# GMichailov/Flash-Attention-CUDA-C

Hardware: AMD Instinct MI355X
Metric: fwd attention TFLOP/s/GPU (bf16, seq=4096, d=128) + % MFMA peak (higher is better)
Workload: dtype bf16

## Files before the change

flash-attention-cuda-c_amd/csrc/computers.hip.h:

```cpp
#pragma once

#include "slot_engine.hip.h"

namespace fa {

template <int R>
struct Scores {
    f32x16 s[R][2];
};

template <class C>
struct WaveCompute : SlotEngine<WaveCompute<C>, C> {
    static constexpr int D = C::D, ESZ = C::ESZ, R = 1;
    static constexpr int KS = D / 16;
    static constexpr int DB = D / 32;
    static constexpr int NA = 2 * KS, NB = 4 * DB;
    static constexpr int SA = NA * R, SB = NB * R;
    static constexpr int MPF = ESZ == 1 ? 2 : 1;
    static constexpr int NF = NA / MPF;
    static constexpr int FPH = NF / 2;
    static constexpr int NPRE = C::NPRE < NF ? C::NPRE : NF;
    static constexpr int VPRE = C::VPRE;
    static constexpr int GROUPS = R, RG = 32, LOG_RG = 5, FPG = FPH;
    static constexpr int NE = 32 * R;
    static constexpr int SPAN = SA + (3 * SB) / 4;
    using G = TileGeom<D, ESZ>;
    using Stage = std::conditional_t<C::MIX, MixStage<D, C::NWAVES>,
                  std::conditional_t<C::DMA, DmaStage<D, C::NWAVES, false, true>,
                                     std::conditional_t<C::DMA_K8, HybridStageFp8<D, C::NWAVES>, BufStage<D, ESZ, C::NWAVES, C::PAD>>>>;
    using ScoresT = Scores<R>;
    static constexpr int NL = Stage::NL, NW = Stage::NW;

    u32x4 qf[R][FPH];
    f32x16 o[R][DB];
    float m[R];
    float l[R];
    u32x4 kf[NPRE];
    bf16x8 vf[VPRE + 1];
    uint32_t pw[R][16];
    float sum_a[R], sum_b[R], mx_a[R], mx_b[R], p_even, p_last;
    bool need;
    unsigned long long t_mid = 0, t_end = 0;

    __device__ __forceinline__ void init() {
#pragma unroll
        for (int r = 0; r < R; ++r) {
#pragma unroll
            for (int i = 0; i < DB; ++i)
#pragma unroll
                for (int k = 0; k < 16; ++k) o[r][i][k] = 0.f;
            m[r] = -INFINITY;
            l[r] = 0.f;
        }
// ... 14 lines not shown
            if constexpr ((F & 1) && SUB == MPF - 1) acc = mfma_32x32x64_fp8_unit_scale(kprev, kfrag, qf[RG][(F - 1) % FPH], q, acc);
        } else {
            static_assert(ESZ == 2, "the non-scaled form is for bf16 inputs");
            acc = mfma_32x32x16(__builtin_bit_cast(bf16x8, kfrag), __builtin_bit_cast(bf16x8, q), acc);
        }
    }
    __device__ __forceinline__ static void zero(Scores<R>& n) {
#pragma unroll
        for (int r = 0; r < R; ++r)
#pragma unroll
            for (int k = 0; k < 16; ++k) { n.s[r][0][k] = 0.f; n.s[r][1][k] = 0.f; }
    }

    template <int I = 0>
    __device__ __forceinline__ void qk_all(lds_ptr kimg, int kbase, Scores<R>& n) {
        if constexpr (I == 0) zero(n);
        if constexpr (I < SA) {
            constexpr int f = I / (MPF * R), sub = (I % (MPF * R)) / R, rg = I % R;
            if constexpr (I % (MPF * R) == 0) kf[f % 2] = k_read(kimg, kbase, f);
            qk_mfma<f, sub, rg>(kf[(f + 1) % 2], kf[f % 2], n);
            qk_all<I + 1>(kimg, kbase, n);
        }
    }

    __device__ __forceinline__ void mask(Scores<R>& n, int kv0, int q_row0, int S, int lane) const {
        const int k0 = kv0 + 4 * (lane >> 5);
#pragma unroll
        for (int r = 0; r < R; ++r) {
            const int qi = q_row0 + 32 * r + (lane & 31);
            const int lim = C::CAUSAL ? (qi < S - 1 ? qi : S - 1) : S - 1;
#pragma unroll
            for (int k = 0; k < 16; ++k) {
                n.s[r][0][k] = (k0 + acc_row(k, 0)) > lim ? -INFINITY : n.s[r][0][k];
                n.s[r][1][k] = (k0 + 32 + acc_row(k, 0)) > lim ? -INFINITY : n.s[r][1][k];
            }
        }
// ... 98 lines not shown
                constexpr int vn = v + VPRE;
                vf[vn % (VPRE + 1)] = v_frag(v_cur, vbase, vn / DB, vn % DB);
            }
            this->template exp_slot<SA + J, F16W>(cur, c);
            if constexpr (TRACK && J < SB / 2) max3_slot<J>(nxt);
            if constexpr (TRACK && J == SB / 2) this->decide(c);
            this->template write_in_slot<J, F16W>(st, wr_slot);
            __builtin_amdgcn_sched_barrier(0);
            slots_b<TRACK, J + 1, F16W>(st, wr_slot, v_cur, vbase, c, cur, nxt);
        }
    }

    __host__ __device__ static constexpr int tail_elem_slot(int E) { return (E / 8 - 1) * DB + (E % 8) * DB / 8; }
    template <int E, bool F16W = false>
    __device__ __forceinline__ void tail_pre(Stage& st, int t_load, lds_ptr v_cur, int vbase, float c, const Scores<R>& cur) {
        static_assert(R == 1 && NL <= 8 && VPRE <= DB, "tail step: one row group, the lead-in carries every piece");
        if constexpr (E < 8) {
            if constexpr (E < VPRE) vf[E % (VPRE + 1)] = v_frag(v_cur, vbase, E / DB, E % DB);
            if constexpr (E < NL) st.template load<E, F16W>(t_load);
            this->template exp_elem<E, F16W>(cur, c);
            tail_pre<E + 1, F16W>(st, t_load, v_cur, vbase, c, cur);
        }
    }
    template <int J, int ST, int E = 8, bool F16W = false>
    __device__ __forceinline__ void tail_exp(const Scores<R>& cur, float c) {
        if constexpr (E < 8 * (ST / DB)) {
            if constexpr (tail_elem_slot(E) == J) this->template exp_elem<E, F16W>(cur, c);
            tail_exp<J, ST, E + 1, F16W>(cur, c);
        }
    }
    template <int J, int J1, int ST, bool F16W = false>
    __device__ __forceinline__ void slots_t(lds_ptr v_cur, int vbase, float c, const Scores<R>& cur) {
        if constexpr (J < J1) {
            constexpr int s4 = J / DB, db = J % DB;
            if constexpr (F16W) o[0][db] = mfma_32x32x16(__builtin_bit_cast(f16x8, vf[J % (VPRE + 1)]), __builtin_bit_cast(f16x8, p_frag(0, s4)), o[0][db]);
            else o[0][db] = mfma_32x32x16(vf[J % (VPRE + 1)], p_frag(0, s4), o[0][db]);
            if constexpr (J + VPRE < ST) {
                constexpr int vn = J + VPRE;
                vf[vn % (VPRE + 1)] = v_frag(v_cur, vbase, vn / DB, vn % DB);
            }
            tail_exp<J, ST, 8, F16W>(cur, c);
            __builtin_amdgcn_sched_barrier(0);
            slots_t<J + 1, J1, ST, F16W>(v_cur, vbase, c, cur);
        }
    }
    __device__ __forceinline__ void begin_tail(Stage& st, lds_ptr wr_slot) {
        st.set_dst(wr_slot);
#pragma unroll
        for (int r = 0; r < R; ++r) sum_a[r] = sum_b[r] = 0.f;
    }

    __device__ __forceinline__ void begin_tile(Stage& st, lds_ptr wr_slot, Scores<R>& nxt) {
        st.set_dst(wr_slot);
#pragma unroll
        for (int r = 0; r < R; ++r) {
            sum_a[r] = sum_b[r] = 0.f;
            mx_a[r] = mx_b[r] = -INFINITY;
        }
// ... 17 lines not shown

    __device__ __forceinline__ bool not_finite() const {
        float acc[4] = {0.f, 0.f, 0.f, 0.f};
#pragma unroll
        for (int r = 0; r < R; ++r) {
            acc[0] = fmaf(l[r], 0.f, acc[0]);
#pragma unroll
            for (int i = 0; i < DB; ++i)
#pragma unroll
                for (int k = 0; k < 16; ++k) acc[k & 3] = fmaf(o[r][i][k], 0.f, acc[k & 3]);
        }
        const float a = (acc[0] + acc[1]) + (acc[2] + acc[3]);
        return a != a;
    }

    template <typename OutT>
    __device__ __forceinline__ void store_o_lds(lds_ptr region, char* Oh, float* lse_head, int64_t oS_bytes, int row0, int S,
                                                int lane, int orow_bytes = D * 2) {
        static_assert(sizeof(OutT) == 2, "LDS epilogue is for bf16 / f16 outputs");
        constexpr int ROWB = D * 2, CHUNKS = ROWB / 16;
        const int q = lane & 31, h = lane >> 5;
#pragma unroll
        for (int r = 0; r < R; ++r) {
            const float l_tot = sum_both_halves(l[r]);
            this->store_lse(lse_head, l_tot, r, row0, S, lane);
            const float inv = 1.0f / l_tot;
#pragma unroll
            for (int db = 0; db < DB; ++db)
#pragma unroll
                for (int g4 = 0; g4 < 4; ++g4) {
                    const int d0 = 32 * db + 8 * g4 + 4 * h;
                    const float a = o[r][db][4 * g4 + 0] * inv, b = o[r][db][4 * g4 + 1] * inv;
                    const float c2 = o[r][db][4 * g4 + 2] * inv, e = o[r][db][4 * g4 + 3] * inv;
                    u32x2 v;
                    if constexpr (__is_same(OutT, __bf16)) v = u32x2{pack_bf16(a, b), pack_bf16(c2, e)};
                    else v = u32x2{pack_f16(a, b), pack_f16(c2, e)};
                    const int chunk = (d0 * 2) >> 4, half8 = (d0 * 2) & 8;
                    *reinterpret_cast<FA_LDS u32x2*>(region + (32 * r + q) * ROWB + (((chunk ^ q) & (CHUNKS - 1)) << 4) + half8) = v;
                }
        }
        __builtin_amdgcn_s_waitcnt(0xc07f);
        constexpr int ROWS_PER_INST = 64 / CHUNKS;
        const int rr = lane / CHUNKS, cc = lane % CHUNKS;
        if (!C::PAD && row0 + 32 * R <= S) {
            u32x4 v[32 * R / ROWS_PER_INST];
#pragma unroll
            for (int i = 0; i < 32 * R / ROWS_PER_INST; ++i) {
                const int row = i * ROWS_PER_INST + rr;
                v[i] = *reinterpret_cast<FA_LDS const u32x4*>(region + row * ROWB + (((cc ^ row) & (CHUNKS - 1)) << 4));
            }
#pragma unroll
            for (int i = 0; i < 32 * R / ROWS_PER_INST; ++i)
                store_global_b128<C::O_CACHE>(Oh + (int64_t)(row0 + i * ROWS_PER_INST + rr) * oS_bytes + cc * 16, v[i]);
            return;
        }
#pragma unroll
        for (int i = 0; i < 32 * R / ROWS_PER_INST; ++i) {
            const int row = i * ROWS_PER_INST + rr;
            const u32x4 v = *reinterpret_cast<FA_LDS const u32x4*>(region + row * ROWB + (((cc ^ row) & (CHUNKS - 1)) << 4));
            if (row0 + row < S && (!C::PAD || cc * 16 < orow_bytes))
                *reinterpret_cast<u32x4*>(Oh + (int64_t)(row0 + row) * oS_bytes + cc * 16) = v;
        }
    }
    template <typename OutT>
    __device__ __forceinline__ void store_o_lds32(lds_ptr region, char* Oh, float* lse_head, int64_t oS_bytes, int row0, int S,
                                                  int lane, int orow_bytes = D * 4) {
        static_assert(sizeof(OutT) == 4, "for fp32 outputs");
        const int q = lane & 31, h = lane >> 5;
        float inv[R];
#pragma unroll
        for (int r = 0; r < R; ++r) {
            const float l_tot = sum_both_halves(l[r]);
            this->store_lse(lse_head, l_tot, r, row0, S, lane);
            inv[r] = 1.0f / l_tot;
        }
        const int rr = lane >> 4, cc = lane & 15;
#pragma unroll
        for (int hf = 0; hf < D / 64; ++hf) {
            if (hf > 0) __builtin_amdgcn_s_waitcnt(0xc07f);
#pragma unroll
            for (int r = 0; r < R; ++r)
#pragma unroll
                for (int dd = 0; dd < 2; ++dd)
#pragma unroll
                    for (int g4 = 0; g4 < 4; ++g4) {
                        const int db = 2 * hf + dd, cidx = 8 * dd + 2 * g4 + h;
                        const f32x4 v = {o[r][db][4 * g4 + 0] * inv[r], o[r][db][4 * g4 + 1] * inv[r],
                                         o[r][db][4 * g4 + 2] * inv[r], o[r][db][4 * g4 + 3] * inv[r]};
                        *reinterpret_cast<FA_LDS f32x4*>(region + (32 * r + q) * 256 + (((cidx ^ q) & 15) << 4)) = v;
                    }
            __builtin_amdgcn_s_waitcnt(0xc07f);
// ... 21 lines not shown
```

flash-attention-cuda-c_amd/csrc/kernel_bf16.hip.h:

```cpp
#pragma once

#include "computers.hip.h"
#include "computers16.hip.h"

#include <type_traits>

namespace fa {

struct Opt {
    bool stamp = false;
    bool pad = false;
    int m16 = -1;
    int sum_mfma = -1;
    int waves = 8;
    bool p_f16 = false;
    bool mix = false;
    int kv_clamp = -1;
    int q_nt = -1;
    int tail = -1;
    int tail_half = -1;
};

template <int D_, bool CAUSAL_, typename OutT_, int ESZ_ = 2, Opt O = Opt{}>
struct KernelCfg {
    static constexpr int D = D_;
    static constexpr bool CAUSAL = CAUSAL_;
    using OutT = OutT_;
    static constexpr int ESZ = ESZ_;
    static constexpr bool STAMP = O.stamp, PAD = O.pad;
    static constexpr bool PRIO_A = true;
    static constexpr int O_CACHE = CAUSAL_ ? 2 : 0;
    static constexpr int Q_CACHE = (O.q_nt < 0 ? CAUSAL_ : O.q_nt != 0) ? 2 : 0;
    static constexpr bool KV_CLAMP = CAUSAL_ && O.kv_clamp != 0;
    static constexpr bool TAIL = ESZ_ == 2 && O.m16 == 0 && (O.tail < 0 ? CAUSAL_ && O.mix : O.tail != 0);
    static constexpr bool TAIL_HALF = TAIL && CAUSAL_ && O.tail_half != 0;
    static constexpr bool COALESCED_Q = D_ == 128 && !O.pad;
    static constexpr bool MXQK = ESZ_ == 1;
    static constexpr bool M16 = (O.m16 < 0 ? true : O.m16 != 0) && ESZ_ == 2;
    static constexpr bool SUM_MFMA = M16 && (O.sum_mfma < 0 ? true : O.sum_mfma != 0);
    static constexpr bool VALU_FIRST = !M16;
    static constexpr bool P_F16 = M16 && O.p_f16;
    static constexpr bool LATE_ADD = !M16;
    static constexpr bool DMA = ESZ_ == 2 && !O.pad && !O.p_f16;
    static constexpr bool MIX = O.mix && DMA;
    static_assert(!O.mix || (ESZ_ == 2 && !O.pad && !O.p_f16 && (O.m16 == 0 || O.sum_mfma == 0)),
                  "the mixed-precision kernels are the LDS-DMA kernels (16x16x32 engine: with fp32 row sums)");
    static constexpr bool DMA_K8 = ESZ_ == 1 && D_ == 128 && !O.pad && O.waves == 8;
    static constexpr int NPRE = 4;
    static constexpr int VPRE = 2;
    static constexpr int THR = 8;
    static constexpr int NWAVES = O.waves;
    static_assert(NWAVES == 8 || NWAVES == 4, "8 or 4 waves");
    static constexpr int QBLK = 32 * NWAVES;
    static constexpr int RING = 3;
    static constexpr int RING_BYTES = RING * TileGeom<D_, ESZ_>::SLOT;
    static constexpr int EP_OFF = (DMA || DMA_K8) ? TileGeom<D_, ESZ_>::SLOT : 0;
    static constexpr int EP_NEED = EP_OFF + (sizeof(OutT_) == 2 ? QBLK * D_ * 2 : QBLK * 256);
    static constexpr int FLAG_OFF = EP_NEED > RING_BYTES ? EP_NEED : RING_BYTES;
    static constexpr int LDS_BYTES = FLAG_OFF + 64;
    static_assert(LDS_BYTES <= 163840, "160 KiB of LDS per CU");
};

template <int D, bool CAUSAL, typename OutT, int ESZ = 2, bool STAMP = false, bool PAD = false, bool LSE = false>
using ProdCfg = KernelCfg<D, CAUSAL, OutT, ESZ, Opt{.stamp = STAMP, .pad = PAD, .m16 = CAUSAL ? 0 : -1, .sum_mfma = LSE ? 0 : -1}>;
// ... 6 lines not shown
    u32x4 a = *reinterpret_cast<FA_LDS const u32x4*>(flags);
    uint32_t r = a[0] | a[1] | a[2] | a[3];
    if constexpr (NWAVES == 8) {
        const u32x4 b = *reinterpret_cast<FA_LDS const u32x4*>(flags + 16);
        r |= b[0] | b[1] | b[2] | b[3];
    }
    return __builtin_amdgcn_readfirstlane(r) != 0;
}

template <int D, typename OutT, bool STAMP = false>
using MixCfg = KernelCfg<D, true, OutT, 2, Opt{.stamp = STAMP, .m16 = 0, .mix = true}>;

template <class C>
using WaveComputeOf = std::conditional_t<C::M16, WaveCompute16<C>, WaveCompute<C>>;

template <class C, bool TRACK, bool F16W = C::P_F16>
__device__ __forceinline__ bool attention_pass(const Params& p, WaveComputeOf<C>& w, typename WaveComputeOf<C>::Stage& st, lds_ptr smem,
                                               int n_tiles, int my_tiles, int q_row0, int lane,
                                               unsigned long long (&acc)[24], bool tile0_in_flight) {
    using G = TileGeom<C::D, C::ESZ>;
    constexpr bool CAUSAL = C::CAUSAL;
    constexpr int KVBLK = 64, SLOT = G::SLOT, KT = G::K_TILE;
    const int S = p.Sk;
    unsigned long long tp0 = 0, tp1 = 0, tp2 = 0;
    if constexpr (C::STAMP) tp0 = cycle_stamp();
    w.init();
    using WC = WaveComputeOf<C>;
    constexpr int KBLK = (G::ROWB / 16) * 128;
    const int kbase = WC::Stage::K_DMA ? (C::M16 ? kd16_read_base(lane, KBLK) : kd_read_base(lane, KBLK)) : (C::M16 ? k16_read_base(lane) : k_read_base(lane));
    const int vbase = C::M16 ? v16_read_base<C::D>(lane) : v_read_base(lane);
    const float c = p.scale_log2;
    auto needs_mask = [&](int t) { return (CAUSAL && t * KVBLK + KVBLK - 1 > q_row0) || (t * KVBLK + KVBLK > S); };
    typename WC::ScoresT sA, sB;

    if (!tile0_in_flight) st.template load_all_into<F16W>(0, smem);
    st.template write_all<F16W>(smem);
    unsigned long long tw0 = 0;
    if constexpr (C::STAMP) tw0 = cycle_stamp();
    st.wait_all();
    if constexpr (C::STAMP) acc[16] += cycle_stamp() - tw0;
    __syncthreads();
    st.template load_all_into<F16W>(1, smem + SLOT);
    constexpr int AHEAD = C::RING - 1;
    if constexpr (C::STAMP) tp1 = cycle_stamp();
    if (my_tiles > 0) {
        w.qk_all(smem, kbase, sA);
        if (needs_mask(0)) w.mask(sA, 0, q_row0, S, lane);
        w.first_max(sA, c);
    }
    st.template write_all<F16W>(smem + SLOT);
    st.wait_all();
    __syncthreads();
    if constexpr (C::STAMP) { tp2 = cycle_stamp(); acc[8] += tp1 - tp0; acc[9] += tp2 - tp1; }

// ... 89 lines not shown
        Vh = (const char*)p.V + (b * p.vB + hk * p.vH) * ESZ;
        Oh = (char*)p.O + (b * p.oB + h * p.oH) * (int64_t)sizeof(typename C::OutT);
        lse_head = p.lse ? p.lse + (int64_t)g * p.S : nullptr;
        q_row0 = qb * QBLK + wave * WROWS;
        const int q_end = min(p.S, (qb + 1) * QBLK);
        const int k_tiles = (p.Sk + KVBLK - 1) / KVBLK;
        n_tiles = C::CAUSAL ? min(k_tiles, (q_end + KVBLK - 1) / KVBLK) : k_tiles;
        wave_live = q_row0 < p.S;
        my_tiles = !wave_live ? 0 : (C::CAUSAL ? min(n_tiles, (q_row0 + WROWS - 1) / KVBLK + 1) : n_tiles);
    }
    __device__ __forceinline__ int kv_rows(int Sk) const { return C::KV_CLAMP ? min(Sk, 64 * n_tiles) : Sk; }
};

template <class C, bool F16W>
__device__ __forceinline__ void run_passes(const Params& p, WaveComputeOf<C>& w, typename WaveComputeOf<C>::Stage& st, lds_ptr smem,
                                           const UnitCtx<C>& u, int lane, unsigned long long (&acc)[24]) {
    if (!attention_pass<C, false, F16W>(p, w, st, smem, u.n_tiles, u.my_tiles, u.q_row0, lane, acc, true)) return;
    if constexpr (F16W) {
        if (!attention_pass<C, true, true>(p, w, st, smem, u.n_tiles, u.my_tiles, u.q_row0, lane, acc, false)) return;
    }
    attention_pass<C, true, false>(p, w, st, smem, u.n_tiles, u.my_tiles, u.q_row0, lane, acc, false);
}

enum class Kind { ALL, ONE };
template <class C, Kind KIND>
__device__ __forceinline__ bool next_unit(const UnitList& L, int& round, int& g, int& qb) {
    if constexpr (KIND == Kind::ALL) return work_unit<C>(L, round, g, qb);
    else {
        g = L.units;
        qb = L.qb0;
        return round == 0;
    }
// ... 15 lines not shown
    constexpr int WROWS = 32;

    UnitCtx<C> cur;
    cur.set(p, g, qb, wave);
    WaveComputeOf<C> w;
    typename WaveComputeOf<C>::Stage st;
    const int row_bytes = C::PAD ? p.d * ESZ : D * ESZ, orow_bytes = C::PAD ? p.d * (int)sizeof(OutT) : D * (int)sizeof(OutT);
    st.init(cur.Kh, cur.Vh, kSb, vSb, cur.kv_rows(Sk), wave, lane, row_bytes);
    if (C::MIX ? cur.early : C::P_F16) st.template load_all_into<true>(0, smem);
    else st.template load_all_into<false>(0, smem);
    if constexpr (C::COALESCED_Q) w.load_q_rows(cur.Qh, qSb, cur.q_row0, S, lane);
    else w.load_q(cur.Qh, qSb, cur.q_row0, S, lane, row_bytes);
    unsigned long long acc[24] = {0, 0, 0, 0, 0, 0, 0, 0, 0, 0, 0, 0, 0, 0, 0, 0, 0, 0, 0, 0, 0, 0, 0, 0};
    if constexpr (C::STAMP) acc[12] = cycle_stamp() - t_kernel0;

    while (true) {
        unsigned long long t_q0 = 0;
        if constexpr (C::STAMP) t_q0 = cycle_stamp();
        w.pin_q();
        if constexpr (C::COALESCED_Q) {
            using G = TileGeom<D, ESZ>;
            static_assert(G::SLOT + C::QBLK * D * ESZ <= C::LDS_BYTES, "Q staging regions must fit behind slot 0");
            int lane_q = lane;
            asm volatile("" : "+v"(lane_q));
            w.q_rows_to_fragments(smem + G::SLOT + wave * (WROWS * D * ESZ), lane_q);
            w.pin_q();
        }
        if constexpr (C::STAMP) acc[7] += cycle_stamp() - t_q0;

        int lane_p = lane;
        asm volatile("" : "+v"(lane_p));
        if (C::MIX ? cur.early : C::P_F16) {
            if constexpr (C::MIX || C::P_F16) run_passes<C, true>(p, w, st, smem, cur, lane_p, acc);
        } else {
            run_passes<C, false>(p, w, st, smem, cur, lane_p, acc);
        }

        unsigned long long t_nx0 = 0;
        if constexpr (C::STAMP) t_nx0 = cycle_stamp();
        UnitCtx<C> nxt;
        ++round;
        const bool more = next_unit<C, KIND>(L, round, g, qb);
        if (more) {
            nxt.set(p, g, qb, wave);
            st.init(nxt.Kh, nxt.Vh, kSb, vSb, nxt.kv_rows(Sk), wave, lane, row_bytes);
            if (C::MIX ? nxt.early : C::P_F16) st.template load_all_into<true>(0, smem);
            else st.template load_all_into<false>(0, smem);
            int lane_n = lane;
            asm volatile("" : "+v"(lane_n));
            if constexpr (C::COALESCED_Q) w.load_q_rows(nxt.Qh, qSb, nxt.q_row0, S, lane_n);
            else w.load_q(nxt.Qh, qSb, nxt.q_row0, S, lane_n, row_bytes);
            __builtin_amdgcn_sched_barrier(0);
        }

        unsigned long long t_ep0 = 0;
        if constexpr (C::STAMP) { t_ep0 = cycle_stamp(); acc[13] += t_ep0 - t_nx0; }
        int lane_e = lane;
        asm volatile("" : "+v"(lane_e));
        if constexpr (sizeof(OutT) == 2) {
            static_assert(C::EP_OFF + C::QBLK * D * 2 <= C::LDS_BYTES, "epilogue regions must fit the ring");
            if (cur.wave_live)
                w.template store_o_lds<OutT>(smem + C::EP_OFF + wave * (WROWS * D * 2), cur.Oh, cur.lse_head, oSb, cur.q_row0, S, lane_e, orow_bytes);
        } else {
            static_assert(C::EP_OFF + C::QBLK * 64 * 4 <= C::LDS_BYTES, "epilogue regions must fit the ring");
            if (cur.wave_live)
                w.template store_o_lds32<OutT>(smem + C::EP_OFF + wave * (WROWS * 256), cur.Oh, cur.lse_head, oSb, cur.q_row0, S, lane_e, orow_bytes);
        }
        if constexpr (C::STAMP) acc[4] += cycle_stamp() - t_ep0;
        if (!more) break;
        unsigned long long t_b0 = 0;
        if constexpr (C::STAMP) t_b0 = cycle_stamp();
        if constexpr (!C::DMA) __syncthreads();
        if constexpr (C::STAMP) acc[15] += cycle_stamp() - t_b0;
        cur = nxt;
    }
    if constexpr (C::STAMP) {
        const unsigned long long t_tail0 = cycle_stamp();
        asm volatile("s_waitcnt vmcnt(0)" ::: "memory");
        const unsigned long long t_end = cycle_stamp();
        acc[14] = t_end - t_tail0;
        acc[0] = t_end - t_kernel0;
        const unsigned long long t_real1 = realtime_stamp();
// ... 40 lines not shown
```

flash-attention-cuda-c_amd/csrc/slot_engine.hip.h:

```cpp
#pragma once

#include "loaders.hip.h"

namespace fa {

template <class W, class C>
struct SlotEngine {
    __device__ __forceinline__ W& self() { return *static_cast<W*>(this); }

    __host__ __device__ static constexpr int elem_slot(int E) { return E * W::SPAN / W::NE; }
    __host__ __device__ static constexpr int load_slot(int n) { return 1 + 2 * n; }
    __host__ __device__ static constexpr int wstep() { return 2 * W::NW <= W::SB / 2 + 1 ? 2 : 1; }
    template <int SLOT, bool F16W = false, int N = 0, class St>
    __device__ __forceinline__ void load_in_slot(St& st, int t_load) {
        if constexpr (N < W::NL) {
            if constexpr (load_slot(N) == SLOT) st.template load<N, F16W>(t_load);
            load_in_slot<SLOT, F16W, N + 1>(st, t_load);
        }
    }
    template <int J, bool F16W = false, class St>
    __device__ __forceinline__ void write_in_slot(St& st, lds_ptr wr_slot) {
        constexpr int H = W::SB / 2, WSTEP = wstep();
        static_assert(2 * W::NL <= W::SA && WSTEP * (W::NW - 1) < W::SB - H, "staging does not fit the slot plan");
        if constexpr (J >= H && (J - H) % WSTEP == 0 && (J - H) / WSTEP < W::NW) st.template write<(J - H) / WSTEP, F16W>(wr_slot);
// ... 16 lines not shown
            const char* src = Qh + row * qS_bytes + (lane >> W::LOG_RG) * 16;
#pragma unroll
            for (int u = 0; u < W::FPG; ++u) {
                if constexpr (C::PAD) {
                    w.qf[g][u] = u32x4{0u, 0u, 0u, 0u};
                    if (u * FSTRIDE + (lane >> W::LOG_RG) * 16 < row_bytes) w.qf[g][u] = load_global_b128<C::Q_CACHE>(src + u * FSTRIDE);
                } else {
                    w.qf[g][u] = load_global_b128<C::Q_CACHE>(src + u * FSTRIDE);
                }
            }
        }
    }
    static constexpr int QCH = (C::D * C::ESZ) / 16, QRPI = 64 / QCH;
    __device__ __forceinline__ void load_q_rows(const char* Qh, int64_t qS_bytes, int row0, int S, int lane) {
        static_assert(32 / QRPI == W::GROUPS * W::FPG, "coalesced Q: as many loads as fragments");
#pragma unroll
        for (int i = 0; i < W::GROUPS * W::FPG; ++i) {
            int row = row0 + i * QRPI + lane / QCH;
            row = row < S ? row : S - 1;
            self().qf[i / W::FPG][i % W::FPG] = load_global_b128<C::Q_CACHE>(Qh + row * qS_bytes + (lane % QCH) * 16);
        }
    }
    __device__ __forceinline__ void q_rows_to_fragments(lds_ptr region, int lane) {
        W& w = self();
        constexpr int ROWB = C::D * C::ESZ;
#pragma unroll
        for (int i = 0; i < W::GROUPS * W::FPG; ++i) {
            const int q = i * QRPI + lane / QCH, c = lane % QCH;
            lds_write_b128(region, q * ROWB + (((c ^ q) & (QCH - 1)) << 4), w.qf[i / W::FPG][i % W::FPG]);
        }
        asm volatile("s_waitcnt lgkmcnt(0)" ::: "memory");
#pragma unroll
        for (int g = 0; g < W::GROUPS; ++g)
#pragma unroll
            for (int u = 0; u < W::FPG; ++u) {
                const int q = W::RG * g + (lane & (W::RG - 1)), c = (64 / W::RG) * u + (lane >> W::LOG_RG);
                w.qf[g][u] = __builtin_bit_cast(u32x4, lds_read_b128(region, q * ROWB + (((c ^ q) & (QCH - 1)) << 4)));
            }
    }
    __device__ __forceinline__ void pin_q() {
#pragma unroll
        for (int g = 0; g < W::GROUPS; ++g)
#pragma unroll
            for (int u = 0; u < W::FPG; ++u) asm volatile("" : "+v"(self().qf[g][u]));
    }
// ... 46 lines not shown
            if (has_next && w.need) {
#pragma unroll
                for (int g = 0; g < W::GROUPS; ++g) {
                    const float mn = fmaxf(w.m[g], w.mx_a[g]);
                    const float alpha = fast_exp2(w.m[g] - mn);
                    w.m[g] = mn;
                    w.rescale(g, alpha);
                }
            }
        }
    }

    template <bool HALF, bool F16W, class Sc>
    __device__ __forceinline__ void tail_rest(lds_ptr v_cur, int vbase, float c, const Sc& cur) {
        constexpr int DB = W::DB, ST = (HALF ? 2 : 4) * DB;
        self().template slots_t<DB, ST, ST, F16W>(v_cur, vbase, c, cur);
    }
    template <bool F16W = false, class St, class Sc>
    __device__ __forceinline__ void tail_step(St& st, int t_load, lds_ptr wr_slot, lds_ptr v_cur, int vbase, float c, const Sc& cur, bool half) {
        W& w = self();
        constexpr int DB = W::DB;
        w.begin_tail(st, wr_slot);
        __builtin_amdgcn_sched_barrier(0);
        w.template tail_pre<0, F16W>(st, t_load, v_cur, vbase, c, cur);
        __builtin_amdgcn_sched_barrier(0);
        if constexpr (C::STAMP) w.t_mid = cycle_stamp();
        w.template slots_t<0, DB, 2 * DB, F16W>(v_cur, vbase, c, cur);
        if (half) tail_rest<true, F16W>(v_cur, vbase, c, cur);
        else tail_rest<false, F16W>(v_cur, vbase, c, cur);
        st.template write_all<F16W>(wr_slot);
// ... 12 lines not shown
```

flash-attention-cuda-c_amd/csrc/utils.hip.h:

```cpp
#pragma once

#include <hip/hip_runtime.h>
#include <stdint.h>

namespace fa {

constexpr int WAVE = 64;

typedef __attribute__((ext_vector_type(16))) float f32x16;
typedef __attribute__((ext_vector_type(4))) float f32x4;
typedef __attribute__((ext_vector_type(2))) float f32x2;
typedef __attribute__((ext_vector_type(8))) __bf16 bf16x8;
typedef __attribute__((ext_vector_type(4))) __bf16 bf16x4;
typedef __attribute__((ext_vector_type(8))) _Float16 f16x8;
typedef __attribute__((ext_vector_type(4))) short s16x4;
typedef __attribute__((ext_vector_type(4))) uint32_t u32x4;
typedef __attribute__((ext_vector_type(2))) uint32_t u32x2;
typedef __attribute__((ext_vector_type(8))) int i32x8;

#define FA_LDS __attribute__((address_space(3)))
typedef FA_LDS char* lds_ptr;

__device__ __forceinline__ f32x16 mfma_32x32x16(bf16x8 a, bf16x8 b, f32x16 c) {
    return __builtin_amdgcn_mfma_f32_32x32x16_bf16(a, b, c, 0, 0, 0);
}
__device__ __forceinline__ f32x4 mfma_16x16x32(bf16x8 a, bf16x8 b, f32x4 c) {
    return __builtin_amdgcn_mfma_f32_16x16x32_bf16(a, b, c, 0, 0, 0);
}
__device__ __forceinline__ f32x4 mfma_16x16x32(f16x8 a, f16x8 b, f32x4 c) {
    return __builtin_amdgcn_mfma_f32_16x16x32_f16(a, b, c, 0, 0, 0);
}
__device__ __forceinline__ f32x16 mfma_32x32x16(f16x8 a, f16x8 b, f32x16 c) {
    return __builtin_amdgcn_mfma_f32_32x32x16_f16(a, b, c, 0, 0, 0);
}
__device__ __forceinline__ f32x16 mfma_32x32x16_fp8(uint64_t a, uint64_t b, f32x16 c) {
    return __builtin_amdgcn_mfma_f32_32x32x16_fp8_fp8((long)a, (long)b, c, 0, 0, 0);
// ... 5 lines not shown
    return __builtin_amdgcn_mfma_scale_f32_32x32x64_f8f6f4(a, b, c, 0, 0, 0, 0x7f7f7f7f, 0, 0x7f7f7f7f);
}

__host__ __device__ constexpr int acc_row(int reg, int h) { return (reg & 3) + 8 * (reg >> 2) + 4 * h; }

__device__ __forceinline__ bf16x8 lds_read_b128(lds_ptr base, int byte_off) {
    return *reinterpret_cast<FA_LDS const bf16x8*>(base + byte_off);
}
__device__ __forceinline__ void lds_write_b128(lds_ptr base, int byte_off, u32x4 v) {
    *reinterpret_cast<FA_LDS u32x4*>(base + byte_off) = v;
}
__device__ __forceinline__ s16x4 lds_read_tr16_b64(lds_ptr base, int byte_off) {
    return __builtin_amdgcn_ds_read_tr16_b64_v4i16(reinterpret_cast<FA_LDS s16x4*>(base + byte_off));
}

template <int POLICY>
__device__ __forceinline__ void store_global_b128(void* p, u32x4 v) {
    if constexpr (POLICY == 0) *reinterpret_cast<u32x4*>(p) = v;
    else if constexpr (POLICY == 1) asm volatile("global_store_dwordx4 %0, %1, off sc1\n\ts_nop 1" ::"v"(p), "v"(v) : "memory");
    else if constexpr (POLICY == 2) asm volatile("global_store_dwordx4 %0, %1, off nt\n\ts_nop 1" ::"v"(p), "v"(v) : "memory");
    else asm volatile("global_store_dwordx4 %0, %1, off sc0 sc1\n\ts_nop 1" ::"v"(p), "v"(v) : "memory");
}

template <int POLICY>
__device__ __forceinline__ u32x4 load_global_b128(const void* p) {
    static_assert(POLICY == 0 || POLICY == 2, "load policies: plain or nt");
    if constexpr (POLICY == 0) return *reinterpret_cast<const u32x4*>(p);
    else return __builtin_nontemporal_load(reinterpret_cast<const u32x4*>(p));
}

__device__ __forceinline__ float other_half(float x) {
    const uint32_t u = __float_as_uint(x);
    auto r = __builtin_amdgcn_permlane32_swap(u, u, false, false);
    const bool lo = (threadIdx.x & 32) == 0;
    return __uint_as_float(lo ? r[1] : r[0]);
}
__device__ __forceinline__ float max_both_halves(float x) {
    const uint32_t u = __float_as_uint(x);
    auto r = __builtin_amdgcn_permlane32_swap(u, u, false, false);
    return fmaxf(__uint_as_float(r[0]), __uint_as_float(r[1]));
}
__device__ __forceinline__ float max_all_quarters(float x) {
    const uint32_t u = __float_as_uint(x);
// ... 86 lines not shown
```

Measured before the change: 1088.

## Overlap unit seam: counted vmcnt wait, parked Q rows, strength-reduced row addressing

Adds several seam-level changes enabled by default for causal mix configs. Q rows are parked in LDS early so the wait before the next unit only drains the new K/V loads rather than the outstanding O stores (a counted vmcnt). Q loads and O stores use global address-space pointers stepped per row instead of full 64-bit multiplies. QK^T uses a deeper K-fragment window, and the tail gets its own V prefetch depth. The risks are more register pressure and correctness hazards from the partial waitcnt.

```diff
diff --git a/flash-attention-cuda-c_amd/csrc/computers.hip.h b/flash-attention-cuda-c_amd/csrc/computers.hip.h
--- a/flash-attention-cuda-c_amd/csrc/computers.hip.h
+++ b/flash-attention-cuda-c_amd/csrc/computers.hip.h
@@ -21,6 +21,7 @@
     static constexpr int FPH = NF / 2;
     static constexpr int NPRE = C::NPRE < NF ? C::NPRE : NF;
     static constexpr int VPRE = C::VPRE;
+    static constexpr int TVPRE = C::TAIL_VPRE;
     static constexpr int GROUPS = R, RG = 32, LOG_RG = 5, FPG = FPH;
     static constexpr int NE = 32 * R;
     static constexpr int SPAN = SA + (3 * SB) / 4;
@@ -36,7 +37,7 @@
     float m[R];
     float l[R];
     u32x4 kf[NPRE];
-    bf16x8 vf[VPRE + 1];
+    bf16x8 vf[(TVPRE > VPRE ? TVPRE : VPRE) + 1];
     uint32_t pw[R][16];
     float sum_a[R], sum_b[R], mx_a[R], mx_b[R], p_even, p_last;
     bool need;
@@ -81,12 +82,27 @@
 
     template <int I = 0>
     __device__ __forceinline__ void qk_all(lds_ptr kimg, int kbase, Scores<R>& n) {
-        if constexpr (I == 0) zero(n);
-        if constexpr (I < SA) {
-            constexpr int f = I / (MPF * R), sub = (I % (MPF * R)) / R, rg = I % R;
-            if constexpr (I % (MPF * R) == 0) kf[f % 2] = k_read(kimg, kbase, f);
-            qk_mfma<f, sub, rg>(kf[(f + 1) % 2], kf[f % 2], n);
-            qk_all<I + 1>(kimg, kbase, n);
+        if constexpr (C::QK0_WINDOW && !C::MXQK) {
+            constexpr int f = I / R, rg = I % R;
+            if constexpr (I == 0) {
+                zero(n);
+#pragma unroll
+                for (int i = 0; i < NPRE; ++i) kf[i] = k_read(kimg, kbase, i);
+            }
+            if constexpr (I < SA) {
+                qk_mfma<f, 0, rg>(kf[f % NPRE], kf[f % NPRE], n);
+                if constexpr (rg == R - 1 && f + NPRE < NF) kf[f % NPRE] = k_read(kimg, kbase, f + NPRE);
+                __builtin_amdgcn_sched_barrier(0);
+                qk_all<I + 1>(kimg, kbase, n);
+            }
+        } else {
+            if constexpr (I == 0) zero(n);
+            if constexpr (I < SA) {
+                constexpr int f = I / (MPF * R), sub = (I % (MPF * R)) / R, rg = I % R;
+                if constexpr (I % (MPF * R) == 0) kf[f % 2] = k_read(kimg, kbase, f);
+                qk_mfma<f, sub, rg>(kf[(f + 1) % 2], kf[f % 2], n);
+                qk_all<I + 1>(kimg, kbase, n);
+            }
         }
     }
 
@@ -215,9 +231,10 @@
     __host__ __device__ static constexpr int tail_elem_slot(int E) { return (E / 8 - 1) * DB + (E % 8) * DB / 8; }
     template <int E, bool F16W = false>
     __device__ __forceinline__ void tail_pre(Stage& st, int t_load, lds_ptr v_cur, int vbase, float c, const Scores<R>& cur) {
-        static_assert(R == 1 && NL <= 8 && VPRE <= DB, "tail step: one row group, the lead-in carries every piece");
+        static_assert(R == 1 && NL <= 8 && TVPRE >= 1 && TVPRE <= 8 && TVPRE <= 2 * DB,
+                      "tail step: one row group, the lead-in carries every piece and reads no V^T fragment past k-step 1");
         if constexpr (E < 8) {
-            if constexpr (E < VPRE) vf[E % (VPRE + 1)] = v_frag(v_cur, vbase, E / DB, E % DB);
+            if constexpr (E < TVPRE) vf[E % (TVPRE + 1)] = v_frag(v_cur, vbase, E / DB, E % DB);
             if constexpr (E < NL) st.template load<E, F16W>(t_load);
             this->template exp_elem<E, F16W>(cur, c);
             tail_pre<E + 1, F16W>(st, t_load, v_cur, vbase, c, cur);
@@ -234,15 +251,22 @@
     __device__ __forceinline__ void slots_t(lds_ptr v_cur, int vbase, float c, const Scores<R>& cur) {
         if constexpr (J < J1) {
             constexpr int s4 = J / DB, db = J % DB;
-            if constexpr (F16W) o[0][db] = mfma_32x32x16(__builtin_bit_cast(f16x8, vf[J % (VPRE + 1)]), __builtin_bit_cast(f16x8, p_frag(0, s4)), o[0][db]);
-            else o[0][db] = mfma_32x32x16(vf[J % (VPRE + 1)], p_frag(0, s4), o[0][db]);
-            if constexpr (J + VPRE < ST) {
-                constexpr int vn = J + VPRE;
-                vf[vn % (VPRE + 1)] = v_frag(v_cur, vbase, vn / DB, vn % DB);
+            if constexpr (F16W) o[0][db] = mfma_32x32x16(__builtin_bit_cast(f16x8, vf[J % (TVPRE + 1)]), __builtin_bit_cast(f16x8, p_frag(0, s4)), o[0][db]);
+            else o[0][db] = mfma_32x32x16(vf[J % (TVPRE + 1)], p_frag(0, s4), o[0][db]);
+            if constexpr (J + TVPRE < ST) {
+                constexpr int vn = J + TVPRE;
+                vf[vn % (TVPRE + 1)] = v_frag(v_cur, vbase, vn / DB, vn % DB);
             }
             tail_exp<J, ST, 8, F16W>(cur, c);
             __builtin_amdgcn_sched_barrier(0);
             slots_t<J + 1, J1, ST, F16W>(v_cur, vbase, c, cur);
+        }
+    }
+    template <int ST, int V = 2 * DB>
+    __device__ __forceinline__ void tail_lead(lds_ptr v_cur, int vbase) {
+        if constexpr (V < DB + TVPRE && V < ST) {
+            vf[V % (TVPRE + 1)] = v_frag(v_cur, vbase, V / DB, V % DB);
+            tail_lead<ST, V + 1>(v_cur, vbase);
         }
     }
     __device__ __forceinline__ void begin_tail(Stage& st, lds_ptr wr_slot) {
@@ -290,7 +314,7 @@
         return a != a;
     }
 
-    template <typename OutT>
+    template <typename OutT, int WAY = 0>
     __device__ __forceinline__ void store_o_lds(lds_ptr region, char* Oh, float* lse_head, int64_t oS_bytes, int row0, int S,
                                                 int lane, int orow_bytes = D * 2) {
         static_assert(sizeof(OutT) == 2, "LDS epilogue is for bf16 / f16 outputs");
@@ -318,16 +342,28 @@
         __builtin_amdgcn_s_waitcnt(0xc07f);
         constexpr int ROWS_PER_INST = 64 / CHUNKS;
         const int rr = lane / CHUNKS, cc = lane % CHUNKS;
-        if (!C::PAD && row0 + 32 * R <= S) {
+        if (WAY == 1 || (WAY == 0 && !C::PAD && row0 + 32 * R <= S)) {
             u32x4 v[32 * R / ROWS_PER_INST];
 #pragma unroll
             for (int i = 0; i < 32 * R / ROWS_PER_INST; ++i) {
                 const int row = i * ROWS_PER_INST + rr;
                 v[i] = *reinterpret_cast<FA_LDS const u32x4*>(region + row * ROWB + (((cc ^ row) & (CHUNKS - 1)) << 4));
             }
+            if constexpr (C::ROW_ADD) {
+                static_assert(ROWS_PER_INST == 4 || ROWS_PER_INST == 8, "rows per instruction");
+                global_ptr dst = (global_ptr)Oh + ((int64_t)row0 * oS_bytes + cc * 16 + small_times<(ROWS_PER_INST == 8 ? 3 : 2)>(rr, oS_bytes));
+#pragma unroll
+                for (int i = 0; i < 32 * R / ROWS_PER_INST; ++i) {
+                    store_global_b128<C::O_CACHE, C::WAIT_COUNTED>(dst, v[i]);
+                    if (i + 1 < 32 * R / ROWS_PER_INST) dst = row_step(dst, ROWS_PER_INST * oS_bytes);
+                }
+                if constexpr (C::WAIT_COUNTED) this->template park_q_rows<1>(region, lane);
+                return;
+            }
 #pragma unroll
             for (int i = 0; i < 32 * R / ROWS_PER_INST; ++i)
-                store_global_b128<C::O_CACHE>(Oh + (int64_t)(row0 + i * ROWS_PER_INST + rr) * oS_bytes + cc * 16, v[i]);
+                store_global_b128<C::O_CACHE, C::WAIT_COUNTED>((global_ptr)Oh + ((int64_t)(row0 + i * ROWS_PER_INST + rr) * oS_bytes + cc * 16), v[i]);
+            if constexpr (C::WAIT_COUNTED) this->template park_q_rows<2>(region, lane);
             return;
         }
 #pragma unroll
@@ -337,8 +373,24 @@
             if (row0 + row < S && (!C::PAD || cc * 16 < orow_bytes))
                 *reinterpret_cast<u32x4*>(Oh + (int64_t)(row0 + row) * oS_bytes + cc * 16) = v;
         }
-    }
-    template <typename OutT>
+        if constexpr (C::WAIT_COUNTED) this->template park_q_rows<3>(region, lane);
+    }
+    __device__ __forceinline__ void half_to_lds32(lds_ptr region, int hf, const float (&inv)[R], int q, int h) const {
+        if (hf > 0) __builtin_amdgcn_s_waitcnt(0xc07f);
+#pragma unroll
+        for (int r = 0; r < R; ++r)
+#pragma unroll
+            for (int dd = 0; dd < 2; ++dd)
+#pragma unroll
+                for (int g4 = 0; g4 < 4; ++g4) {
+                    const int db = 2 * hf + dd, cidx = 8 * dd + 2 * g4 + h;
+                    const f32x4 v = {o[r][db][4 * g4 + 0] * inv[r], o[r][db][4 * g4 + 1] * inv[r],
+                                     o[r][db][4 * g4 + 2] * inv[r], o[r][db][4 * g4 + 3] * inv[r]};
+                    *reinterpret_cast<FA_LDS f32x4*>(region + (32 * r + q) * 256 + (((cidx ^ q) & 15) << 4)) = v;
+                }
+        __builtin_amdgcn_s_waitcnt(0xc07f);
+    }
+    template <typename OutT, int WAY = 0>
     __device__ __forceinline__ void store_o_lds32(lds_ptr region, char* Oh, float* lse_head, int64_t oS_bytes, int row0, int S,
                                                   int lane, int orow_bytes = D * 4) {
         static_assert(sizeof(OutT) == 4, "for fp32 outputs");
@@ -351,6 +403,47 @@
             inv[r] = 1.0f / l_tot;
         }
         const int rr = lane >> 4, cc = lane & 15;
+        if constexpr (C::ROW_ADD || C::WAIT_COUNTED) {
+            static_assert(D / 64 <= 2, "fp32 rows of one or two 256-byte halves");
+            if (WAY == 1 || (WAY == 0 && !C::PAD && row0 + 32 * R <= S)) {
+                global_ptr orow[8 * R];
+#pragma unroll
+                for (int hf = 0; hf < D / 64; ++hf) {
+                    half_to_lds32(region, hf, inv, q, h);
+                    f32x4 v[8 * R];
+#pragma unroll
+                    for (int i = 0; i < 8 * R; ++i) v[i] = *reinterpret_cast<FA_LDS const f32x4*>(region + (4 * i + rr) * 256 + (((cc ^ (4 * i + rr)) & 15) << 4));
+#pragma unroll
+                    for (int i = 0; i < 8 * R; ++i) {
+                        if constexpr (C::ROW_ADD) {
+                            if (hf == 0) {
+                                orow[i] = i == 0 ? (global_ptr)Oh + ((int64_t)row0 * oS_bytes + cc * 16 + small_times<2>(rr, oS_bytes)) : row_step(orow[i - 1], 4 * oS_bytes);
+                                store_global_b128<C::O_CACHE, C::WAIT_COUNTED>(orow[i], __builtin_bit_cast(u32x4, v[i]));
+                            } else {
+                                store_global_b128_at<C::O_CACHE, 256, C::WAIT_COUNTED>(orow[i], __builtin_bit_cast(u32x4, v[i]));
+                            }
+                        } else {
+                            store_global_b128<C::O_CACHE, C::WAIT_COUNTED>((global_ptr)Oh + ((int64_t)(row0 + 4 * i + rr) * oS_bytes + hf * 256 + cc * 16), __builtin_bit_cast(u32x4, v[i]));
+                        }
+                    }
+                }
+                if constexpr (C::WAIT_COUNTED) this->template park_q_rows<1>(region, lane);
+            } else {
+#pragma unroll
+                for (int hf = 0; hf < D / 64; ++hf) {
+                    half_to_lds32(region, hf, inv, q, h);
+#pragma unroll
+                    for (int i = 0; i < 8 * R; ++i) {
+                        const int row = 4 * i + rr;
+                        const f32x4 v = *reinterpret_cast<FA_LDS const f32x4*>(region + row * 256 + (((cc ^ row) & 15) << 4));
+                        if (row0 + row < S && (!C::PAD || hf * 256 + cc * 16 < orow_bytes))
+                            *reinterpret_cast<f32x4*>(Oh + (int64_t)(row0 + row) * oS_bytes + hf * 256 + cc * 16) = v;
+                    }
+                }
+                if constexpr (C::WAIT_COUNTED) this->template park_q_rows<2>(region, lane);
+            }
+            return;
+        }
 #pragma unroll
         for (int hf = 0; hf < D / 64; ++hf) {
             if (hf > 0) __builtin_amdgcn_s_waitcnt(0xc07f);
diff --git a/flash-attention-cuda-c_amd/csrc/kernel_bf16.hip.h b/flash-attention-cuda-c_amd/csrc/kernel_bf16.hip.h
--- a/flash-attention-cuda-c_amd/csrc/kernel_bf16.hip.h
+++ b/flash-attention-cuda-c_amd/csrc/kernel_bf16.hip.h
@@ -19,6 +19,10 @@
     int q_nt = -1;
     int tail = -1;
     int tail_half = -1;
+    int row_add = -1;
+    int wait_counted = -1;
+    int qk0_window = -1;
+    int tail_vpre = -1;
 };
 
 template <int D_, bool CAUSAL_, typename OutT_, int ESZ_ = 2, Opt O = Opt{}>
@@ -34,6 +38,13 @@
     static constexpr bool KV_CLAMP = CAUSAL_ && O.kv_clamp != 0;
     static constexpr bool TAIL = ESZ_ == 2 && O.m16 == 0 && (O.tail < 0 ? CAUSAL_ && O.mix : O.tail != 0);
     static constexpr bool TAIL_HALF = TAIL && CAUSAL_ && O.tail_half != 0;
+#ifdef FA_SEAM2_OFF
+    static constexpr bool SEAM2 = false;
+#else
+    static constexpr bool SEAM2 = CAUSAL_ && O.mix;
+#endif
+    static constexpr bool ROW_ADD = O.row_add < 0 ? SEAM2 : O.row_add != 0;
+    static constexpr bool QK0_WINDOW = ESZ_ == 2 && O.m16 == 0 && (O.qk0_window < 0 ? SEAM2 : O.qk0_window != 0);
     static constexpr bool COALESCED_Q = D_ == 128 && !O.pad;
     static constexpr bool MXQK = ESZ_ == 1;
     static constexpr bool M16 = (O.m16 < 0 ? true : O.m16 != 0) && ESZ_ == 2;
@@ -48,6 +59,8 @@
     static constexpr bool DMA_K8 = ESZ_ == 1 && D_ == 128 && !O.pad && O.waves == 8;
     static constexpr int NPRE = 4;
     static constexpr int VPRE = 2;
+    static constexpr int TAIL_VPRE = (TAIL && O.tail_vpre > 0) ? O.tail_vpre : VPRE;
+    static constexpr bool WAIT_COUNTED = DMA && COALESCED_Q && (O.wait_counted < 0 ? SEAM2 : O.wait_counted != 0);
     static constexpr int THR = 8;
     static constexpr int NWAVES = O.waves;
     static_assert(NWAVES == 8 || NWAVES == 4, "8 or 4 waves");
@@ -84,10 +97,16 @@
 template <class C>
 using WaveComputeOf = std::conditional_t<C::M16, WaveCompute16<C>, WaveCompute<C>>;
 
+template <class C>
+struct SeamStores {
+    static constexpr int O = 32 * C::D * (int)sizeof(typename C::OutT) / (64 * 16);
+    static_assert(O + 8 < 64, "vmcnt is a 6-bit count");
+};
+
 template <class C, bool TRACK, bool F16W = C::P_F16>
 __device__ __forceinline__ bool attention_pass(const Params& p, WaveComputeOf<C>& w, typename WaveComputeOf<C>::Stage& st, lds_ptr smem,
                                                int n_tiles, int my_tiles, int q_row0, int lane,
-                                               unsigned long long (&acc)[24], bool tile0_in_flight) {
+                                               unsigned long long (&acc)[24], bool tile0_in_flight, int seam_vm = -1) {
     using G = TileGeom<C::D, C::ESZ>;
     constexpr bool CAUSAL = C::CAUSAL;
     constexpr int KVBLK = 64, SLOT = G::SLOT, KT = G::K_TILE;
@@ -107,7 +126,12 @@
     st.template write_all<F16W>(smem);
     unsigned long long tw0 = 0;
     if constexpr (C::STAMP) tw0 = cycle_stamp();
-    st.wait_all();
+    if constexpr (C::WAIT_COUNTED && !F16W) {
+        if (tile0_in_flight && seam_vm == SeamStores<C>::O) asm volatile("s_waitcnt vmcnt(%0)" ::"n"(SeamStores<C>::O) : "memory");
+        else st.wait_all();
+    } else {
+        st.wait_all();
+    }
     if constexpr (C::STAMP) acc[16] += cycle_stamp() - tw0;
     __syncthreads();
     st.template load_all_into<F16W>(1, smem + SLOT);
@@ -227,8 +251,8 @@
 
 template <class C, bool F16W>
 __device__ __forceinline__ void run_passes(const Params& p, WaveComputeOf<C>& w, typename WaveComputeOf<C>::Stage& st, lds_ptr smem,
-                                           const UnitCtx<C>& u, int lane, unsigned long long (&acc)[24]) {
-    if (!attention_pass<C, false, F16W>(p, w, st, smem, u.n_tiles, u.my_tiles, u.q_row0, lane, acc, true)) return;
+                                           const UnitCtx<C>& u, int lane, unsigned long long (&acc)[24], int seam_vm) {
+    if (!attention_pass<C, false, F16W>(p, w, st, smem, u.n_tiles, u.my_tiles, u.q_row0, lane, acc, true, seam_vm)) return;
     if constexpr (F16W) {
         if (!attention_pass<C, true, true>(p, w, st, smem, u.n_tiles, u.my_tiles, u.q_row0, lane, acc, false)) return;
     }
@@ -274,16 +298,23 @@
     unsigned long long acc[24] = {0, 0, 0, 0, 0, 0, 0, 0, 0, 0, 0, 0, 0, 0, 0, 0, 0, 0, 0, 0, 0, 0, 0, 0};
     if constexpr (C::STAMP) acc[12] = cycle_stamp() - t_kernel0;
 
+    if constexpr (C::WAIT_COUNTED) {
+        using G = TileGeom<D, ESZ>;
+        static_assert(C::EP_OFF == G::SLOT && WROWS * D * ESZ == (sizeof(OutT) == 2 ? WROWS * D * 2 : WROWS * 256), "one region per wave for Q and O");
+        w.park_q_rows(smem + G::SLOT + wave * (WROWS * D * ESZ), lane);
+    }
+    int seam_vm = -1;
     while (true) {
         unsigned long long t_q0 = 0;
         if constexpr (C::STAMP) t_q0 = cycle_stamp();
-        w.pin_q();
+        if constexpr (!C::WAIT_COUNTED) w.pin_q();
         if constexpr (C::COALESCED_Q) {
             using G = TileGeom<D, ESZ>;
             static_assert(G::SLOT + C::QBLK * D * ESZ <= C::LDS_BYTES, "Q staging regions must fit behind slot 0");
             int lane_q = lane;
             asm volatile("" : "+v"(lane_q));
-            w.q_rows_to_fragments(smem + G::SLOT + wave * (WROWS * D * ESZ), lane_q);
+            if constexpr (C::WAIT_COUNTED) w.fragments_from_rows(smem + G::SLOT + wave * (WROWS * D * ESZ), lane_q);
+            else w.q_rows_to_fragments(smem + G::SLOT + wave * (WROWS * D * ESZ), lane_q);
             w.pin_q();
         }
         if constexpr (C::STAMP) acc[7] += cycle_stamp() - t_q0;
@@ -291,9 +322,9 @@
         int lane_p = lane;
         asm volatile("" : "+v"(lane_p));
         if (C::MIX ? cur.early : C::P_F16) {
-            if constexpr (C::MIX || C::P_F16) run_passes<C, true>(p, w, st, smem, cur, lane_p, acc);
+            if constexpr (C::MIX || C::P_F16) run_passes<C, true>(p, w, st, smem, cur, lane_p, acc, seam_vm);
         } else {
-            run_passes<C, false>(p, w, st, smem, cur, lane_p, acc);
+            run_passes<C, false>(p, w, st, smem, cur, lane_p, acc, seam_vm);
         }
 
         unsigned long long t_nx0 = 0;
@@ -301,31 +332,64 @@
         UnitCtx<C> nxt;
         ++round;
         const bool more = next_unit<C, KIND>(L, round, g, qb);
-        if (more) {
-            nxt.set(p, g, qb, wave);
-            st.init(nxt.Kh, nxt.Vh, kSb, vSb, nxt.kv_rows(Sk), wave, lane, row_bytes);
-            if (C::MIX ? nxt.early : C::P_F16) st.template load_all_into<true>(0, smem);
-            else st.template load_all_into<false>(0, smem);
-            int lane_n = lane;
-            asm volatile("" : "+v"(lane_n));
-            if constexpr (C::COALESCED_Q) w.load_q_rows(nxt.Qh, qSb, nxt.q_row0, S, lane_n);
-            else w.load_q(nxt.Qh, qSb, nxt.q_row0, S, lane_n, row_bytes);
-            __builtin_amdgcn_sched_barrier(0);
-        }
-
         unsigned long long t_ep0 = 0;
-        if constexpr (C::STAMP) { t_ep0 = cycle_stamp(); acc[13] += t_ep0 - t_nx0; }
-        int lane_e = lane;
-        asm volatile("" : "+v"(lane_e));
-        if constexpr (sizeof(OutT) == 2) {
-            static_assert(C::EP_OFF + C::QBLK * D * 2 <= C::LDS_BYTES, "epilogue regions must fit the ring");
-            if (cur.wave_live)
-                w.template store_o_lds<OutT>(smem + C::EP_OFF + wave * (WROWS * D * 2), cur.Oh, cur.lse_head, oSb, cur.q_row0, S, lane_e, orow_bytes);
+        if constexpr (C::WAIT_COUNTED) {
+            if (more) {
+                nxt.set(p, g, qb, wave);
+                st.init(nxt.Kh, nxt.Vh, kSb, vSb, nxt.kv_rows(Sk), wave, lane, row_bytes);
+                if (C::MIX ? nxt.early : C::P_F16) st.template load_all_into<true>(0, smem);
+                else st.template load_all_into<false>(0, smem);
+            }
+            auto seam_way = [&]<int WAY>() {
+                asm volatile("; unit seam, way %0" ::"n"(WAY) : "memory");
+                if (more) {
+                    int lane_n = lane;
+                    asm volatile("" : "+v"(lane_n));
+                    if constexpr (C::COALESCED_Q) w.load_q_rows(nxt.Qh, qSb, nxt.q_row0, S, lane_n);
+                    else w.load_q(nxt.Qh, qSb, nxt.q_row0, S, lane_n, row_bytes);
+                    __builtin_amdgcn_sched_barrier(0);
+                }
+                if constexpr (C::STAMP) { t_ep0 = cycle_stamp(); acc[13] += t_ep0 - t_nx0; }
+                int lane_e = lane;
+                asm volatile("" : "+v"(lane_e));
+                if constexpr (sizeof(OutT) == 2) {
+                    static_assert(C::EP_OFF + C::QBLK * D * 2 <= C::LDS_BYTES, "epilogue regions must fit the ring");
+                    w.template store_o_lds<OutT, WAY>(smem + C::EP_OFF + wave * (WROWS * D * 2), cur.Oh, cur.lse_head, oSb, cur.q_row0, S, lane_e, orow_bytes);
+                } else {
+                    static_assert(C::EP_OFF + C::QBLK * 64 * 4 <= C::LDS_BYTES, "epilogue regions must fit the ring");
+                    w.template store_o_lds32<OutT, WAY>(smem + C::EP_OFF + wave * (WROWS * 256), cur.Oh, cur.lse_head, oSb, cur.q_row0, S, lane_e, orow_bytes);
+                }
+            };
+            if (!C::PAD && cur.q_row0 + WROWS <= S) seam_way.template operator()<1>();
+            else seam_way.template operator()<2>();
         } else {
-            static_assert(C::EP_OFF + C::QBLK * 64 * 4 <= C::LDS_BYTES, "epilogue regions must fit the ring");
-            if (cur.wave_live)
-                w.template store_o_lds32<OutT>(smem + C::EP_OFF + wave * (WROWS * 256), cur.Oh, cur.lse_head, oSb, cur.q_row0, S, lane_e, orow_bytes);
-        }
+            if (more) {
+                nxt.set(p, g, qb, wave);
+                st.init(nxt.Kh, nxt.Vh, kSb, vSb, nxt.kv_rows(Sk), wave, lane, row_bytes);
+                if (C::MIX ? nxt.early : C::P_F16) st.template load_all_into<true>(0, smem);
+                else st.template load_all_into<false>(0, smem);
+                int lane_n = lane;
+                asm volatile("" : "+v"(lane_n));
+                if constexpr (C::COALESCED_Q) w.load_q_rows(nxt.Qh, qSb, nxt.q_row0, S, lane_n);
+                else w.load_q(nxt.Qh, qSb, nxt.q_row0, S, lane_n, row_bytes);
+                __builtin_amdgcn_sched_barrier(0);
+            }
+
+            if constexpr (C::STAMP) { t_ep0 = cycle_stamp(); acc[13] += t_ep0 - t_nx0; }
+            int lane_e = lane;
+            asm volatile("" : "+v"(lane_e));
+            if constexpr (sizeof(OutT) == 2) {
+                static_assert(C::EP_OFF + C::QBLK * D * 2 <= C::LDS_BYTES, "epilogue regions must fit the ring");
+                if (cur.wave_live)
+                    w.template store_o_lds<OutT>(smem + C::EP_OFF + wave * (WROWS * D * 2), cur.Oh, cur.lse_head, oSb, cur.q_row0, S, lane_e, orow_bytes);
+            } else {
+                static_assert(C::EP_OFF + C::QBLK * 64 * 4 <= C::LDS_BYTES, "epilogue regions must fit the ring");
+                if (cur.wave_live)
+                    w.template store_o_lds32<OutT>(smem + C::EP_OFF + wave * (WROWS * 256), cur.Oh, cur.lse_head, oSb, cur.q_row0, S, lane_e, orow_bytes);
+            }
+        }
+        if constexpr (C::WAIT_COUNTED)
+            seam_vm = (!C::PAD && cur.q_row0 + WROWS <= S) ? SeamStores<C>::O : -1;
         if constexpr (C::STAMP) acc[4] += cycle_stamp() - t_ep0;
         if (!more) break;
         unsigned long long t_b0 = 0;
diff --git a/flash-attention-cuda-c_amd/csrc/slot_engine.hip.h b/flash-attention-cuda-c_amd/csrc/slot_engine.hip.h
--- a/flash-attention-cuda-c_amd/csrc/slot_engine.hip.h
+++ b/flash-attention-cuda-c_amd/csrc/slot_engine.hip.h
@@ -54,6 +54,20 @@
     static constexpr int QCH = (C::D * C::ESZ) / 16, QRPI = 64 / QCH;
     __device__ __forceinline__ void load_q_rows(const char* Qh, int64_t qS_bytes, int row0, int S, int lane) {
         static_assert(32 / QRPI == W::GROUPS * W::FPG, "coalesced Q: as many loads as fragments");
+        if constexpr (C::ROW_ADD) {
+            static_assert((QRPI & (QRPI - 1)) == 0 && QRPI <= 8, "rows per instruction: a power of two");
+            constexpr int RBITS = QRPI == 8 ? 3 : QRPI == 4 ? 2 : QRPI == 2 ? 1 : 0;
+            const int row = row0 + lane / QCH;
+            global_ptr src = (global_ptr) const_cast<char*>(Qh) + ((int64_t)row0 * qS_bytes + (lane % QCH) * 16 + small_times<RBITS>(lane / QCH, qS_bytes));
+            const global_ptr last = (global_ptr) const_cast<char*>(Qh) + ((int64_t)(S - 1) * qS_bytes + (lane % QCH) * 16);
+            const int64_t step = QRPI * qS_bytes;
+#pragma unroll
+            for (int i = 0; i < W::GROUPS * W::FPG; ++i) {
+                self().qf[i / W::FPG][i % W::FPG] = load_global_b128<C::Q_CACHE>(row + i * QRPI < S ? src : last);
+                if (i + 1 < W::GROUPS * W::FPG) src = row_step(src, step);
+            }
+            return;
+        }
 #pragma unroll
         for (int i = 0; i < W::GROUPS * W::FPG; ++i) {
             int row = row0 + i * QRPI + lane / QCH;
@@ -62,6 +76,11 @@
         }
     }
     __device__ __forceinline__ void q_rows_to_fragments(lds_ptr region, int lane) {
+        park_q_rows(region, lane);
+        fragments_from_rows(region, lane);
+    }
+    template <int WAY = 0>
+    __device__ __forceinline__ void park_q_rows(lds_ptr region, int lane) {
         W& w = self();
         constexpr int ROWB = C::D * C::ESZ;
 #pragma unroll
@@ -69,6 +88,11 @@
             const int q = i * QRPI + lane / QCH, c = lane % QCH;
             lds_write_b128(region, q * ROWB + (((c ^ q) & (QCH - 1)) << 4), w.qf[i / W::FPG][i % W::FPG]);
         }
+        if constexpr (WAY > 0) asm volatile("; Q rows parked, way %0" ::"n"(WAY) : "memory");
+    }
+    __device__ __forceinline__ void fragments_from_rows(lds_ptr region, int lane) {
+        W& w = self();
+        constexpr int ROWB = C::D * C::ESZ;
         asm volatile("s_waitcnt lgkmcnt(0)" ::: "memory");
 #pragma unroll
         for (int g = 0; g < W::GROUPS; ++g)
@@ -145,6 +169,7 @@
     template <bool HALF, bool F16W, class Sc>
     __device__ __forceinline__ void tail_rest(lds_ptr v_cur, int vbase, float c, const Sc& cur) {
         constexpr int DB = W::DB, ST = (HALF ? 2 : 4) * DB;
+        self().template tail_lead<ST>(v_cur, vbase);
         self().template slots_t<DB, ST, ST, F16W>(v_cur, vbase, c, cur);
     }
     template <bool F16W = false, class St, class Sc>
diff --git a/flash-attention-cuda-c_amd/csrc/utils.hip.h b/flash-attention-cuda-c_amd/csrc/utils.hip.h
--- a/flash-attention-cuda-c_amd/csrc/utils.hip.h
+++ b/flash-attention-cuda-c_amd/csrc/utils.hip.h
@@ -20,6 +20,8 @@
 
 #define FA_LDS __attribute__((address_space(3)))
 typedef FA_LDS char* lds_ptr;
+#define FA_GLOBAL __attribute__((address_space(1)))
+typedef FA_GLOBAL char* global_ptr;
 
 __device__ __forceinline__ f32x16 mfma_32x32x16(bf16x8 a, bf16x8 b, f32x16 c) {
     return __builtin_amdgcn_mfma_f32_32x32x16_bf16(a, b, c, 0, 0, 0);
@@ -55,12 +57,37 @@
     return __builtin_amdgcn_ds_read_tr16_b64_v4i16(reinterpret_cast<FA_LDS s16x4*>(base + byte_off));
 }
 
-template <int POLICY>
-__device__ __forceinline__ void store_global_b128(void* p, u32x4 v) {
-    if constexpr (POLICY == 0) *reinterpret_cast<u32x4*>(p) = v;
+__device__ __forceinline__ u32x4* as_u32x4(const void*);
+__device__ __forceinline__ FA_GLOBAL u32x4* as_u32x4(const FA_GLOBAL void*);
+
+template <int POLICY, bool COUNTED = false, class P>
+__device__ __forceinline__ void store_global_b128(P* p, u32x4 v) {
+    if constexpr (POLICY == 0) *(decltype(as_u32x4(p)))p = v;
+    else if constexpr (POLICY == 2 && COUNTED) __builtin_nontemporal_store(v, (decltype(as_u32x4(p)))p);
     else if constexpr (POLICY == 1) asm volatile("global_store_dwordx4 %0, %1, off sc1\n\ts_nop 1" ::"v"(p), "v"(v) : "memory");
     else if constexpr (POLICY == 2) asm volatile("global_store_dwordx4 %0, %1, off nt\n\ts_nop 1" ::"v"(p), "v"(v) : "memory");
     else asm volatile("global_store_dwordx4 %0, %1, off sc0 sc1\n\ts_nop 1" ::"v"(p), "v"(v) : "memory");
+}
+
+template <int POLICY, int OFFSET, bool COUNTED = false>
+__device__ __forceinline__ void store_global_b128_at(global_ptr p, u32x4 v) {
+    static_assert((POLICY == 0 || POLICY == 2) && OFFSET > 0 && OFFSET < 4096, "plain or nt, the instruction's 12-bit offset");
+    if constexpr (POLICY == 0) *(FA_GLOBAL u32x4*)(p + OFFSET) = v;
+    else if constexpr (COUNTED) __builtin_nontemporal_store(v, (FA_GLOBAL u32x4*)(p + OFFSET));
+    else asm volatile("global_store_dwordx4 %0, %1, off offset:%2 nt\n\ts_nop 1" ::"v"(p), "v"(v), "n"(OFFSET) : "memory");
+}
+
+__device__ __forceinline__ global_ptr row_step(global_ptr p, int64_t stride_bytes) {
+    p += stride_bytes;
+    asm volatile("" : "+v"(p));
+    return p;
+}
+template <int BITS>
+__device__ __forceinline__ int64_t small_times(int r, int64_t stride_bytes) {
+    int64_t a = 0;
+#pragma unroll
+    for (int b = 0; b < BITS; ++b) a += ((r >> b) & 1) ? (int64_t)((uint64_t)stride_bytes << b) : (int64_t)0;
+    return a;
 }
 
 template <int POLICY>
@@ -68,6 +95,13 @@
     static_assert(POLICY == 0 || POLICY == 2, "load policies: plain or nt");
     if constexpr (POLICY == 0) return *reinterpret_cast<const u32x4*>(p);
     else return __builtin_nontemporal_load(reinterpret_cast<const u32x4*>(p));
+}
+
+template <int POLICY>
+__device__ __forceinline__ u32x4 load_global_b128(const FA_GLOBAL void* p) {
+    static_assert(POLICY == 0 || POLICY == 2, "load policies: plain or nt");
+    if constexpr (POLICY == 0) return *(const FA_GLOBAL u32x4*)p;
+    else return __builtin_nontemporal_load((const FA_GLOBAL u32x4*)p);
 }
 
 __device__ __forceinline__ float other_half(float x) {
```

Result: no change. 1090 (median of 6 runs) (+0.1%).
